# wenxiaoshuai/Points-Matching

Measured on AMD Instinct MI355X. Metric: descriptor-pair distances/s (BF-L2 2-NN + ratio stage); RANSAC hypotheses/s in `ransac`, higher is better.
Workload: dtype f32

## Files before the change

### points_matching_amd/csrc/ransac_a_fused.hip

```cpp
#include "affine_core.hpp"
#include "ransac_fused_kernels.hpp"

namespace pm_ransac {
namespace {

using namespace pm_affine;

constexpr int RA_SYNC_WORD = 12;

template <int MODEL>
struct AModel {
    static constexpr int MIN_PTS = Traits<MODEL>::MIN_PTS;
    static constexpr bool SHARD_OUT = false;
    static constexpr int OUT_WORDS = 6;
    static constexpr bool CANDIDATES = false;

    template <typename DIAG>
    static __device__ __forceinline__ bool solve(const pm_points_view& v, const int* __restrict__ offs, int n, uint64_t seed,
                                                 uint64_t h, double (&A)[9])
    {
        int idx[MIN_PTS];
        sample<MODEL>(seed, h, n, idx);
        double x1[MIN_PTS], y1[MIN_PTS], x2[MIN_PTS], y2[MIN_PTS];
#pragma unroll
        for (int i = 0; i < MIN_PTS; ++i) {
            float2 a, b;
            view_point(v, offs, idx[i], a, b);
            x1[i] = static_cast<double>(a.x); y1[i] = static_cast<double>(a.y);
            x2[i] = static_cast<double>(b.x); y2[i] = static_cast<double>(b.y);
        }
        if constexpr (MODEL == FULL) return solve3(x1, y1, x2, y2, A);
        else return solve2(x1, y1, x2, y2, A);
    }

    static __device__ __forceinline__ void inlier_pk(const ModelS& m, f32x2 x, f32x2 y, f32x2 xp, f32x2 yp, float thr2, bool& ia,
                                                     bool& ib)
    {
        const f32x2 u = sfma_out<0>(m.q03, x, sfma_in<0, 1>(m.q12, y));
        const f32x2 v = sfma_out<1>(m.q03, x, sfma_in<0, 1>(m.q45, y));
        const f32x2 du = u - xp, dv = v - yp;
        const f32x2 lhs = __builtin_elementwise_fma(du, du, dv * dv);
// ... 24 lines not shown
```

### points_matching_amd/csrc/ransac_core.hpp

```cpp
#pragma once
#include "pm_common.hpp"

namespace pm_ransac {

struct NoDiag {
    static constexpr bool scalar_fma = false;
    static __device__ __forceinline__ void phase(int) {}
    static __device__ __forceinline__ void solve(int) {}
};

constexpr int MODEL_STRIDE = 12;

__device__ __forceinline__ uint64_t mix64(uint64_t z)
{
    z = (z ^ (z >> 30)) * 0xBF58476D1CE4E5B9ULL;
    z = (z ^ (z >> 27)) * 0x94D049BB133111EBULL;
    return z ^ (z >> 31);
}

__device__ __forceinline__ void sample8(uint64_t seed, uint64_t h, int n, int (&idx)[8])
{
    const uint64_t stream = mix64(seed ^ 0x9E3779B97F4A7C15ULL) ^ mix64(h + 0xD1B54A32D192ED03ULL);
    int cand[8];
#pragma unroll
    for (int d = 0; d < 8; ++d) {
        const uint64_t r = mix64(stream + static_cast<uint64_t>(d + 1) * 0x9E3779B97F4A7C15ULL);
        cand[d] = static_cast<int>(((r >> 32) * static_cast<uint64_t>(static_cast<uint32_t>(n))) >> 32);
    }
    unsigned dup = 0u;
#pragma unroll
    for (int d = 1; d < 8; ++d)
#pragma unroll
        for (int e = 0; e < d; ++e) dup |= (cand[e] == cand[d] ? 1u : 0u) << d;
#pragma unroll
    for (int s = 0; s < 8; ++s) idx[s] = cand[s];
    if (dup == 0u) return;
#pragma unroll
    for (int s = 0; s < 8; ++s) idx[s] = -1;
    int cnt = 0;
#pragma unroll
    for (int d = 0; d < 8; ++d) {
// ... 315 lines not shown
```

### points_matching_amd/csrc/ransac_e_fused.hip

```cpp
#include "ransac_fused_kernels.hpp"

namespace pm_ransac {
namespace {

constexpr int RE_SYNC_WORD = 16;

struct EModel {
    static constexpr int MIN_PTS = 5;
    static constexpr bool SHARD_OUT = false;
    static constexpr int OUT_WORDS = 9;
    static constexpr bool CANDIDATES = true;

    static __device__ __forceinline__ bool load(const double* __restrict__ cand, int k, double (&E)[9])
    {
        const double* c = cand + 10 * static_cast<size_t>(k);
#pragma unroll
        for (int i = 0; i < 9; ++i) E[i] = c[i];
        return c[9] != 0.0;
    }
    static __device__ __forceinline__ void inlier_pk(const ModelS& m, f32x2 x, f32x2 y, f32x2 xp, f32x2 yp, float thr2, bool& ia,
                                                     bool& ib)
    {
        FModel<PM_ERR_SAMPSON>::inlier_pk(m, x, y, xp, yp, thr2, ia, ib);
    }
    static __device__ __forceinline__ void inlier_x2(const float (&f)[9], f32x2 x, f32x2 y, f32x2 xp, f32x2 yp, float thr2,
                                                     bool& ia, bool& ib)
    {
        FModel<PM_ERR_SAMPSON>::inlier_x2(f, x, y, xp, yp, thr2, ia, ib);
    }
};

}

int ransac_e_enqueue(pm_ctx* ctx, const pm_points_view& vn, const pm_ransac_params* q, const double* d_cand,
                     unsigned long long* d_key, double* d_E, uint8_t* d_mask, int mask_len, int* d_ninl)
{
    return fused_lds_enqueue<EModel>(ctx, vn, q, RE_SYNC_WORD, "ransac_e_fused", d_key, d_E, d_mask, mask_len, d_ninl, d_cand);
}
// ... 3 lines not shown
```

### points_matching_amd/csrc/ransac_fused_kernels.hpp

```cpp
#pragma once
#include <type_traits>

#include "ransac_core.hpp"
#include "ransac_internal.hpp"

namespace pm_ransac {
namespace {

constexpr int RF_THREADS = 256;
constexpr int RF_TEAMS = 2;
constexpr int RF_WG = RF_THREADS * RF_TEAMS;
constexpr int RF_PTS_PER_SLOT = 2 * RF_THREADS;
constexpr int RF_PPT2 = 5;
constexpr int RF_PPT2_BIG = 10;
static_assert(RF_PPT2_BIG <= 10, "score_tile is instantiated for 1..10 slots");

struct RfSlot {
    unsigned long long key;
    double F[9];
    unsigned long long pad[6];
};
static_assert(sizeof(RfSlot) == 128, "slot stride");

struct RfOut {
    int shard;
    unsigned long long* key;
    double* F;
    uint8_t* mask;
    int mask_len;
    int* n_inliers;
    FinalOut* fo;
    union {
        pm_ransac_record* rec;
        const double* cand;
    };
};

// ... 165 lines not shown
            bool ia, ib;
            if constexpr (DIAG::scalar_fma) {
                ia = inlier32<KIND>(fs, X[k][0], Y[k][0], XP[k][0], YP[k][0], thr2);
                ib = inlier32<KIND>(fs, X[k][1], Y[k][1], XP[k][1], YP[k][1], thr2);
            } else {
                inlier_pk_model<KIND>(ms, X[k], Y[k], XP[k], YP[k], thr2, ia, ib);
            }
            va[k] = __ballot(ia);
            vb[k] = __ballot(ib);
        }
        int c = 0;
#pragma unroll
        for (int k = 0; k < KM; ++k) c += __popcll(va[k]) + __popcll(vb[k]);
        if (lane == 0) {
            if (first) cnt[wave][s] = c;
            else __hip_atomic_fetch_add(&cnt[wave][s], c, __ATOMIC_RELAXED, __HIP_MEMORY_SCOPE_WORKGROUP);
        }
    }
}

template <int NWAVES>
__device__ __forceinline__ unsigned long long wg_max_u64(unsigned long long key, unsigned long long* __restrict__ wk, int tid)
{
    key = pm::wave_max_u64(key);
    __syncthreads();
    if ((tid & 63) == 0) wk[tid >> 6] = key;
    __syncthreads();
    unsigned long long k = wk[0];
#pragma unroll
    for (int w = 1; w < NWAVES; ++w) k = wk[w] > k ? wk[w] : k;
    return k;
}

template <int KIND, int PPT2, typename DIAG>
__global__ __launch_bounds__(RF_WG) void ransac_fused(pm_points_view v, uint64_t seed, int64_t hyp_begin, int nh, int hb,
                                                           float thr2, RfSlot* __restrict__ slots, int* __restrict__ ticket,
                                                           RfOut out)
{
    __shared__ __attribute__((aligned(16))) float s_mdl[RF_HB_MAX][12];
    __shared__ double s_m64[RF_HB_MAX][9];
    __shared__ int s_cnt[RF_THREADS / 64][RF_HB_MAX];
    __shared__ int s_offs[PM_MAX_PARTS + 1];
    __shared__ unsigned long long s_wk[RF_WG / 64];
    __shared__ double s_F64[9];
    __shared__ int s_role;
    __shared__ int s_wc[RF_THREADS / 64];

    const int tid = threadIdx.x, lane = tid & 63, wave = tid >> 6;
    const int team = tid / RF_THREADS, ttid = tid % RF_THREADS, twave = wave % (RF_THREADS / 64);
    DIAG::phase(0);
    int n;
    if (v.parts == 1) {
        n = view_count1(v);
    } else {
        view_offsets(v, s_offs, tid);
        __syncthreads();
        n = s_offs[v.parts];
    }
    DIAG::phase(1);

    constexpr int RF_TILE = RF_PTS_PER_SLOT * PPT2;
    const int ntiles = n > RF_TILE ? (n + RF_TILE - 1) / RF_TILE : 1;
    f32x2 X[PPT2], Y[PPT2], XP[PPT2], YP[PPT2];
    const float nanv = __builtin_nanf("");
    auto load_tile = [&](int t) -> int {
        const int base = t * RF_TILE;
        int kmax = (n - base + RF_PTS_PER_SLOT - 1) / RF_PTS_PER_SLOT;
        kmax = kmax < 0 ? 0 : (kmax > PPT2 ? PPT2 : kmax);
#pragma unroll
// ... 24 lines not shown

    const int h0 = static_cast<int>(blockIdx.x) * hb;
    const int hcount = nh - h0 < hb ? nh - h0 : hb;
    if (tid < hcount) {
        double F[9];
        bool ok = false;
#pragma unroll
        for (int i = 0; i < 9; ++i) F[i] = 0.0;
        if (n >= 8) ok = hyp_model_view<DIAG>(v, s_offs, n, seed, static_cast<uint64_t>(hyp_begin + h0 + tid), F);
#pragma unroll
        for (int i = 0; i < 9; ++i) { s_mdl[tid][i] = static_cast<float>(F[i]); s_m64[tid][i] = F[i]; }
        s_mdl[tid][9] = ok ? 1.f : 0.f;
        s_mdl[tid][10] = 0.f; s_mdl[tid][11] = 0.f;
    }
    DIAG::phase(3);
    int kmax = load_tile(0);
    __syncthreads();
    DIAG::phase(4);

    for (int t = 0; t < ntiles; ++t) {
        if (t > 0) kmax = load_tile(t);
        switch (kmax) {
#define PM_CASE(KM_) case KM_: score_tile<KIND, PPT2, (KM_ <= PPT2 ? KM_ : PPT2), DIAG>(s_mdl, s_cnt, hcount, X, Y, XP, YP, thr2, t == 0, lane, twave, team); break;
            PM_CASE(1) PM_CASE(2) PM_CASE(3) PM_CASE(4) PM_CASE(5) PM_CASE(6) PM_CASE(7) PM_CASE(8) PM_CASE(9) PM_CASE(10)
#undef PM_CASE
            default:
                if (team == 0) for (int s = lane; s < hcount; s += 64) s_cnt[twave][s] = t == 0 ? 0 : s_cnt[twave][s];
                break;
        }
    }
    DIAG::phase(5);
    __syncthreads();

    unsigned long long key = 0ull;
    if (tid < hcount && s_mdl[tid][9] != 0.f) {
        int c = 0;
#pragma unroll
        for (int w = 0; w < RF_THREADS / 64; ++w) c += s_cnt[w][tid];
        key = (static_cast<unsigned long long>(static_cast<uint32_t>(c)) << 32) |
              static_cast<unsigned long long>(0xFFFFFFFFu - static_cast<uint32_t>(hyp_begin + h0 + tid));
    }
    const unsigned long long kbest = wg_max_u64<RF_WG / 64>(key, s_wk, tid);
    if (wave == 0) {
        const int sb = kbest ? static_cast<int>(static_cast<int64_t>(0xFFFFFFFFu - static_cast<uint32_t>(kbest)) - hyp_begin) - h0 : 0;
        RfSlot* sl = slots + blockIdx.x;
        if (lane < 9) __hip_atomic_store(&sl->F[lane], kbest ? s_m64[sb][lane] : 0.0, __ATOMIC_RELAXED, __HIP_MEMORY_SCOPE_AGENT);
        if (lane == 9) __hip_atomic_store(&sl->key, kbest, __ATOMIC_RELAXED, __HIP_MEMORY_SCOPE_AGENT);
        asm volatile("s_waitcnt vmcnt(0)" ::: "memory");
        if (lane == 0) {
            const int tk = __hip_atomic_fetch_add(ticket, 1, __ATOMIC_RELAXED, __HIP_MEMORY_SCOPE_AGENT);
            s_role = tk == static_cast<int>(gridDim.x) - 1 ? 1 : 0;
        }
    }
    __syncthreads();
    DIAG::phase(6);
    if (s_role == 0) { DIAG::phase(9); return; }

    if (tid == 0) __hip_atomic_store(ticket, 0, __ATOMIC_RELAXED, __HIP_MEMORY_SCOPE_AGENT);
    unsigned long long kb = 0ull;
    double fb[9];
#pragma unroll
    for (int i = 0; i < 9; ++i) fb[i] = 0.0;
    for (int j = tid; j < static_cast<int>(gridDim.x); j += RF_WG) {
        const unsigned long long kj = __hip_atomic_load(&slots[j].key, __ATOMIC_RELAXED, __HIP_MEMORY_SCOPE_AGENT);
        double fj[9];
#pragma unroll
        for (int i = 0; i < 9; ++i) fj[i] = __hip_atomic_load(&slots[j].F[i], __ATOMIC_RELAXED, __HIP_MEMORY_SCOPE_AGENT);
        if (kj > kb) {
            kb = kj;
#pragma unroll
            for (int i = 0; i < 9; ++i) fb[i] = fj[i];
        }
    }
    const unsigned long long kwin = wg_max_u64<RF_WG / 64>(kb, s_wk, tid);
    const bool ok = kwin != 0ull && n >= 8;
    if (tid < 9) s_F64[tid] = 0.0;
    __syncthreads();
    if (ok && kb == kwin) {
#pragma unroll
        for (int i = 0; i < 9; ++i) s_F64[i] = fb[i];
    }
    __syncthreads();
    DIAG::phase(7);
    if (out.shard) {
        if (tid < 9) out.rec->F[tid] = s_F64[tid];
        if (tid == 9) out.rec->key = ok ? kwin : 0ull;
        return;
    }
    if (tid < 9) {
        if (out.F) out.F[tid] = s_F64[tid];
        if (out.fo) { out.fo->F[tid] = s_F64[tid]; out.fo->F32[tid] = static_cast<float>(s_F64[tid]); }
    }
    if (tid == 9) {
        *out.key = ok ? kwin : 0ull;
        if (out.fo) out.fo->valid = ok ? 1 : 0;
    }
    float fw[9];
#pragma unroll
    for (int i = 0; i < 9; ++i) fw[i] = static_cast<float>(s_F64[i]);
    int mine = 0;
    if (team == 0) {
        for (int t = 0; t < ntiles; ++t) {
            if (ntiles > 1) kmax = load_tile(t);
#pragma unroll
            for (int k = 0; k < PPT2; ++k) {
                if (k < kmax) {
// ... 97 lines not shown
#pragma unroll
            for (int h = 0; h < NH; ++h) s_cnt[ss[h]] += c[h];
        }
    } else {
        ModelS ms[NH];
        int c[NH];
#pragma unroll
        for (int h = 0; h < NH; ++h) {
            const float* m = s_mdl[ss[h]];
            ms[h] = model_to_sgprs(*reinterpret_cast<const f32x4v*>(m), *reinterpret_cast<const f32x4v*>(m + 4),
                                   *reinterpret_cast<const f32x2*>(m + 8));
            c[h] = 0;
        }
        for (int slot = 0; slot < kslots; ++slot) {
            const f32x2 x = pp[0], y = pp[64], xp = pp[128], yp = pp[192];
            pp += 256;
#pragma unroll
            for (int h = 0; h < NH; ++h) {
                bool ia, ib;
                MODEL::inlier_pk(ms[h], x, y, xp, yp, thr2, ia, ib);
                c[h] += __popcll(__ballot(ia)) + __popcll(__ballot(ib));
            }
        }
        if (lane == 0) {
#pragma unroll
            for (int h = 0; h < NH; ++h) s_cnt[ss[h]] += c[h];
        }
    }
}

template <typename MODEL, typename DIAG>
__global__ __launch_bounds__(RL_THREADS) void ransac_fused_lds(pm_points_view v, uint64_t seed, int64_t hyp_begin, int nh, int hb,
                                                               float thr2, int tile_slots, RfSlot* __restrict__ slots,
                                                               int* __restrict__ ticket, RfOut out)
{
    using G = typename GeomOf<MODEL>::type;
    extern __shared__ __attribute__((aligned(16))) f32x2 s_pts[];
    __shared__ __attribute__((aligned(16))) float s_mdl[RF_HB_MAX][G::MW];
    __shared__ double s_m64[RF_HB_MAX][G::WORDS];
    __shared__ int s_cnt[RF_HB_MAX];
    __shared__ int s_offs[PM_MAX_PARTS + 1];
    __shared__ unsigned long long s_wk[RL_WAVES];
    __shared__ double s_F64[G::WORDS];
    __shared__ int s_role;
    __shared__ int s_wc[RL_WAVES];

    const int tid = threadIdx.x, lane = tid & 63, wave = tid >> 6;
    DIAG::phase(0);
    int n;
    if (v.parts == 1) {
        n = view_count1(v);
    } else {
        view_offsets(v, s_offs, tid);
        __syncthreads();
        n = s_offs[v.parts];
    }
    DIAG::phase(1);
    const int tile_pts = tile_slots * RL_SLOT_PTS;
    const int ntiles = n > tile_pts ? (n + tile_pts - 1) / tile_pts : 1;
    const float nanv = __builtin_nanf("");
    auto load_pair = [&](int base, int slot, int l) {
        const int i0 = base + 2 * (64 * slot + l);
        if constexpr (G::OWN) {
            MODEL::load_pair(v, n, i0, s_pts + static_cast<size_t>(slot) * G::PLANES * 64 + l);
        } else {
            float2 a0 = {nanv, nanv}, b0 = a0, a1 = a0, b1 = a0;
            if (v.parts == 1) {
// ... 71 lines not shown
        if constexpr (MODEL::CANDIDATES) {
            const int sk = wave + RL_WAVES * lane;
            unsigned long long live = __ballot(sk < hcount && s_mdl[sk < hcount ? sk : 0][G::FLAG] != 0.f);
            while (live) {
                int ss[4];
                int k = 0;
#pragma unroll
                for (int h = 0; h < 4; ++h) {
                    ss[h] = wave;
                    if (live) {
                        ss[h] = wave + RL_WAVES * static_cast<int>(__builtin_ctzll(live));
                        live &= live - 1;
                        k = h + 1;
                    }
                }
                if (k == 4) score_lds_ids<MODEL, 4, G>(s_mdl, s_cnt, s_pts + lane, kslots, ss, thr2, lane);
                else if (k == 3) score_lds_ids<MODEL, 3, G>(s_mdl, s_cnt, s_pts + lane, kslots, ss, thr2, lane);
                else if (k == 2) score_lds_ids<MODEL, 2, G>(s_mdl, s_cnt, s_pts + lane, kslots, ss, thr2, lane);
                else score_lds_ids<MODEL, 1, G>(s_mdl, s_cnt, s_pts + lane, kslots, ss, thr2, lane);
            }
        } else {
            for (int s = wave; s < hcount; s += 4 * RL_WAVES) {
                const int left = (hcount - s + RL_WAVES - 1) / RL_WAVES;
                if (left >= 4) score_lds<MODEL, 4>(s_mdl, s_cnt, s_pts + lane, kslots, s, thr2, lane);
                else if (left == 3) score_lds<MODEL, 3>(s_mdl, s_cnt, s_pts + lane, kslots, s, thr2, lane);
                else if (left == 2) score_lds<MODEL, 2>(s_mdl, s_cnt, s_pts + lane, kslots, s, thr2, lane);
                else score_lds<MODEL, 1>(s_mdl, s_cnt, s_pts + lane, kslots, s, thr2, lane);
            }
        }
    }
    DIAG::phase(5);
    __syncthreads();

    unsigned long long key = 0ull;
    if (tid < hcount && s_mdl[tid][G::FLAG] != 0.f)
        key = (static_cast<unsigned long long>(static_cast<uint32_t>(s_cnt[tid])) << 32) |
              static_cast<unsigned long long>(0xFFFFFFFFu - static_cast<uint32_t>(hyp_begin + h0 + tid));
    const unsigned long long kbest = wg_max_u64<RL_WAVES>(key, s_wk, tid);
    if (wave == 0) {
        const int sb = kbest ? static_cast<int>(static_cast<int64_t>(0xFFFFFFFFu - static_cast<uint32_t>(kbest)) - hyp_begin) - h0 : 0;
        double* sf = reinterpret_cast<double*>(slots) + static_cast<size_t>(lane) * gridDim.x + blockIdx.x;
        if (lane < G::WORDS) __hip_atomic_store(sf, kbest ? s_m64[sb][lane] : 0.0, __ATOMIC_RELAXED, __HIP_MEMORY_SCOPE_AGENT);
        if (lane == G::WORDS) __hip_atomic_store(reinterpret_cast<unsigned long long*>(sf), kbest, __ATOMIC_RELAXED, __HIP_MEMORY_SCOPE_AGENT);
        asm volatile("s_waitcnt vmcnt(0)" ::: "memory");
        if (lane == 0) {
            const int tk = __hip_atomic_fetch_add(ticket, 1, __ATOMIC_RELAXED, __HIP_MEMORY_SCOPE_AGENT);
            s_role = tk == static_cast<int>(gridDim.x) - 1 ? 1 : 0;
        }
    }
    __syncthreads();
    DIAG::phase(6);
    if (s_role == 0) { DIAG::phase(9); return; }

    if (tid == 0) __hip_atomic_store(ticket, 0, __ATOMIC_RELAXED, __HIP_MEMORY_SCOPE_AGENT);
    unsigned long long kb = 0ull;
    double fb[G::WORDS];
#pragma unroll
    for (int i = 0; i < G::WORDS; ++i) fb[i] = 0.0;
    for (int j = tid; j < static_cast<int>(gridDim.x); j += RL_THREADS) {
        const double* sf = reinterpret_cast<const double*>(slots) + j;
        const unsigned long long kj = __hip_atomic_load(reinterpret_cast<const unsigned long long*>(sf + G::WORDS * static_cast<size_t>(gridDim.x)),
                                                        __ATOMIC_RELAXED, __HIP_MEMORY_SCOPE_AGENT);
        double fj[G::WORDS];
#pragma unroll
        for (int i = 0; i < G::WORDS; ++i) fj[i] = __hip_atomic_load(sf + i * static_cast<size_t>(gridDim.x), __ATOMIC_RELAXED, __HIP_MEMORY_SCOPE_AGENT);
        if (kj > kb) {
            kb = kj;
#pragma unroll
            for (int i = 0; i < G::WORDS; ++i) fb[i] = fj[i];
        }
    }
    const unsigned long long kwin = wg_max_u64<RL_WAVES>(kb, s_wk, tid);
    const bool ok = kwin != 0ull && n >= MODEL::MIN_PTS;
    if (tid < G::WORDS) s_F64[tid] = 0.0;
    __syncthreads();
    if (ok && kb == kwin) {
#pragma unroll
        for (int i = 0; i < G::WORDS; ++i) s_F64[i] = fb[i];
    }
    __syncthreads();
    DIAG::phase(7);
    if (MODEL::SHARD_OUT && out.shard) {
        if (tid < 9) out.rec->F[tid] = s_F64[tid];
        if (tid == 9) out.rec->key = ok ? kwin : 0ull;
        return;
    }
    if (tid < G::WORDS) {
        if (out.F && (MODEL::OUT_WORDS == G::WORDS || tid < MODEL::OUT_WORDS)) out.F[tid] = s_F64[tid];
        if (MODEL::SHARD_OUT && out.fo) { out.fo->F[tid] = s_F64[tid]; out.fo->F32[tid] = static_cast<float>(s_F64[tid]); }
    }
    if (tid == G::WORDS) {
        *out.key = ok ? kwin : 0ull;
        if (MODEL::SHARD_OUT && out.fo) out.fo->valid = ok ? 1 : 0;
    }
    float fw[G::OWN ? G::MW : 9];
    if constexpr (G::OWN) {
        MODEL::mask_model(out.cand, ok, kwin, hyp_begin, fw);
    } else {
#pragma unroll
        for (int i = 0; i < 9; ++i) fw[i] = static_cast<float>(s_F64[i]);
    }
    int mine = 0;
    for (int t = 0; t < ntiles; ++t) {
        const int kslots = tile_kslots(t);
        if (ntiles > 1) {
            __syncthreads();
            for (int slot = wave; slot < kslots; slot += RL_WAVES) load_pair(t * tile_pts, slot, lane);
            __syncthreads();
        }
        for (int slot = wave; slot < kslots; slot += RL_WAVES) {
            const f32x2* pp = s_pts + static_cast<size_t>(slot) * (64 * G::PLANES) + lane;
            bool ia, ib;
            if constexpr (G::OWN) {
                f32x2 op[G::PLANES];
#pragma unroll
                for (int q = 0; q < G::PLANES; ++q) op[q] = pp[64 * q];
                MODEL::inlier_x2(fw, op, thr2, ia, ib);
            } else {
                MODEL::inlier_x2(fw, pp[0], pp[64], pp[128], pp[192], thr2, ia, ib);
            }
            ia = ia && ok; ib = ib && ok;
            const int i0 = t * tile_pts + 2 * (64 * slot + lane);
            if (i0 < out.mask_len) out.mask[i0] = ia ? 1 : 0;
            if (i0 + 1 < out.mask_len) out.mask[i0 + 1] = ib ? 1 : 0;
            mine += __popcll(__ballot(ia)) + __popcll(__ballot(ib));
        }
    }
    if (lane == 0) s_wc[wave] = mine;
    const int covered = n > 0 ? (n + RL_SLOT_PTS - 1) / RL_SLOT_PTS * RL_SLOT_PTS : 0;
    for (int i = covered + tid; i < out.mask_len; i += RL_THREADS) out.mask[i] = 0;
    __syncthreads();
    if (tid == 0) {
        int tot = 0;
#pragma unroll
        for (int w = 0; w < RL_WAVES; ++w) tot += s_wc[w];
        if (out.n_inliers) *out.n_inliers = tot;
        if (MODEL::SHARD_OUT && out.fo) out.fo->n_inliers = tot;
    }
    DIAG::phase(8);
    DIAG::phase(9);
}

int sync_words(pm_ctx* ctx, int** out)
{
    if (!ctx->sync_words) {
        PM_HIP_CHECK(hipMalloc(reinterpret_cast<void**>(&ctx->sync_words), 256));
        PM_HIP_CHECK(hipMemsetAsync(ctx->sync_words, 0, 256, ctx->stream));
    }
    *out = ctx->sync_words;
    return PM_OK;
}

template <typename MODEL, typename DIAG>
int fused_lds_launch(pm_ctx* ctx, const pm_points_view& v, const pm_ransac_params* p, int nwg, int hb, RfSlot* slots,
                     int* ticket, const RfOut& out)
{
    using G = typename GeomOf<MODEL>::type;
    const long long cap_total = static_cast<long long>(v.parts) * v.cap;
    const long long need = (cap_total + RL_SLOT_PTS - 1) / RL_SLOT_PTS;
    const int tile_slots = static_cast<int>(need < 1 ? 1 : (need > G::MAX_SLOTS ? G::MAX_SLOTS : need));
    const size_t lds = static_cast<size_t>(tile_slots) * G::PLANES * 64 * sizeof(f32x2);
    static bool attr_done_dev[PM_MAX_DEVICES] = {};
    if (!attr_done_dev[ctx->device]) {
        PM_HIP_CHECK(hipFuncSetAttribute(reinterpret_cast<const void*>(&ransac_fused_lds<MODEL, DIAG>),
                                         hipFuncAttributeMaxDynamicSharedMemorySize,
                                         G::MAX_SLOTS * G::PLANES * 64 * static_cast<int>(sizeof(f32x2))));
        attr_done_dev[ctx->device] = true;
    }
    const float thr2 = p->thresh_px * p->thresh_px;
    hipLaunchKernelGGL((ransac_fused_lds<MODEL, DIAG>), dim3(nwg), dim3(RL_THREADS), lds, ctx->stream, v, p->seed, p->hyp_begin,
                       static_cast<int>(p->hyp_end - p->hyp_begin), hb, thr2, tile_slots, slots, ticket, out);
    PM_HIP_CHECK(hipGetLastError());
    return PM_OK;
}

template <typename MODEL>
int fused_lds_enqueue(pm_ctx* ctx, const pm_points_view& v, const pm_ransac_params* p, int sync_word, const char* timer,
                      unsigned long long* d_key, double* d_model, uint8_t* d_mask, int mask_len, int* d_ninl,
                      const double* d_cand = nullptr)
{
    const long long nh = p->hyp_end - p->hyp_begin;
    const int hb = fused_hb(ctx, nh);
    const int nwg = static_cast<int>((nh + hb - 1) / hb);
    RfSlot* slots = static_cast<RfSlot*>(pm::arena_take(ctx, sizeof(RfSlot) * static_cast<size_t>(nwg)));
    PM_REQUIRE(slots, PM_E_NOMEM, "scratch arena too small");
    int* sync = nullptr;
    int rc = sync_words(ctx, &sync);
    if (rc != PM_OK) return rc;
    RfOut out{};
    out.key = d_key; out.F = d_model; out.mask = d_mask; out.mask_len = mask_len; out.n_inliers = d_ninl;
    out.cand = d_cand;
    pm::ScopedKernelTime t(ctx, timer);
    return fused_lds_launch<MODEL, NoDiag>(ctx, v, p, nwg, hb, slots, sync + sync_word, out);
}

template <typename DIAG>
int fused_launch_t(pm_ctx* ctx, const pm_points_view& v, const pm_ransac_params* p, int shard, pm_ransac_record* d_rec,
                 unsigned long long* d_key, double* d_F, uint8_t* d_mask, int mask_len, int* d_ninl, FinalOut** fo_out)
{
    const long long nh = p->hyp_end - p->hyp_begin;
    const long long cap_total = static_cast<long long>(v.parts) * v.cap;
    PM_REQUIRE(nh >= 1, PM_E_INVALID, "fused_launch: empty hypothesis range");
    PM_REQUIRE(nh <= 0x7FFFFFFFLL, PM_E_INVALID, "a single launch takes at most 2^31 - 1 hypothesis ids: split the range");
    const int hb = fused_hb(ctx, nh);
    const int nwg = static_cast<int>((nh + hb - 1) / hb);
    RfSlot* slots = static_cast<RfSlot*>(pm::arena_take(ctx, sizeof(RfSlot) * static_cast<size_t>(nwg)));
    FinalOut* fo = static_cast<FinalOut*>(pm::arena_take(ctx, sizeof(FinalOut)));
    PM_REQUIRE(slots && fo, PM_E_NOMEM, "scratch arena too small");
    int* sync = nullptr;
    int rc = sync_words(ctx, &sync);
    if (rc != PM_OK) return rc;
    RfOut out{};
    out.shard = shard;
    out.key = d_key; out.F = d_F; out.mask = d_mask; out.mask_len = mask_len; out.n_inliers = d_ninl;
    out.fo = fo_out ? fo : nullptr;
    out.rec = d_rec;
    if (fo_out) *fo_out = fo;
    const float thr2 = p->thresh_px * p->thresh_px;
    pm::ScopedKernelTime t(ctx, "ransac_fused");
    if (ctx->opts[PM_OPT_RANSAC_FORM] != 1) {
        if (p->error_kind == PM_ERR_SAMPSON) return fused_lds_launch<FModel<PM_ERR_SAMPSON>, DIAG>(ctx, v, p, nwg, hb, slots, sync, out);
        return fused_lds_launch<FModel<PM_ERR_SYM_EPIPOLAR>, DIAG>(ctx, v, p, nwg, hb, slots, sync, out);
    }
#define PM_RF(KIND_, PPT2_)                                                                                              \
    hipLaunchKernelGGL((ransac_fused<KIND_, PPT2_, DIAG>), dim3(nwg), dim3(RF_WG), 0, ctx->stream, v, p->seed, p->hyp_begin, \
                       static_cast<int>(nh), hb, thr2, slots, sync, out)
    const int depth = cap_total <= 2 * RF_PTS_PER_SLOT ? 2 : (cap_total <= RF_PPT2 * RF_PTS_PER_SLOT ? RF_PPT2 : RF_PPT2_BIG);
#define PM_RF_K(KIND_)                                                                   \
    do {                                                                                 \
        if (depth == 2) PM_RF(KIND_, 2);                                                 \
        else if (depth == RF_PPT2) PM_RF(KIND_, RF_PPT2);                                \
        else PM_RF(KIND_, RF_PPT2_BIG);                                                  \
    } while (0)
    if (p->error_kind == PM_ERR_SAMPSON) PM_RF_K(PM_ERR_SAMPSON);
    else PM_RF_K(PM_ERR_SYM_EPIPOLAR);
#undef PM_RF_K
#undef PM_RF
    PM_HIP_CHECK(hipGetLastError());
    return PM_OK;
}

}
}
```

### points_matching_amd/csrc/ransac_h_fused.hip

```cpp
#include "homography_core.hpp"
#include "ransac_fused_kernels.hpp"

namespace pm_ransac {
namespace {

using namespace pm_homog;

constexpr int RH_SYNC_WORD = 8;

struct HModel {
    static constexpr int MIN_PTS = 4;
    static constexpr bool SHARD_OUT = false;
    static constexpr int OUT_WORDS = 9;
    static constexpr bool CANDIDATES = false;

    template <typename DIAG>
    static __device__ __forceinline__ bool solve(const pm_points_view& v, const int* __restrict__ offs, int n, uint64_t seed,
                                                 uint64_t h, double (&H)[9])
    {
        int idx[4];
        sample4(seed, h, n, idx);
        double x1[4], y1[4], x2[4], y2[4];
#pragma unroll
        for (int i = 0; i < 4; ++i) {
            float2 a, b;
            view_point(v, offs, idx[i], a, b);
            x1[i] = static_cast<double>(a.x); y1[i] = static_cast<double>(a.y);
            x2[i] = static_cast<double>(b.x); y2[i] = static_cast<double>(b.y);
        }
        return solve4(x1, y1, x2, y2, H);
    }

    static __device__ __forceinline__ void inlier_pk(const ModelS& m, f32x2 x, f32x2 y, f32x2 xp, f32x2 yp, float thr2, bool& ia,
                                                     bool& ib)
    {
        const f32x2 u = sfma_out<0>(m.q03, x, sfma_in<0, 1>(m.q12, y));
        const f32x2 v = sfma_out<1>(m.q03, x, sfma_in<0, 1>(m.q45, y));
        const f32x2 w = sfma_out<1>(m.q36, x, sfma_in<0, 1>(m.q78, y));
        const f32x2 du = __builtin_elementwise_fma(-xp, w, u);
        const f32x2 dv = __builtin_elementwise_fma(-yp, w, v);
        const f32x2 lhs = __builtin_elementwise_fma(du, du, dv * dv);
// ... 22 lines not shown
```

### points_matching_amd/csrc/ransac_p_fused.hip

```cpp
#include "pnp_core.hpp"
#include "ransac_fused_kernels.hpp"

namespace pm_ransac {
namespace {

using pm_pnp::SLOT_DOUBLES;

constexpr int RP_SYNC_WORD = 20;

struct PnpGeom {
    static constexpr bool OWN = true;
    static constexpr int PLANES = 5, MW = 16, FLAG = 12, WORDS = 12, MAX_SLOTS = 48;
};

__device__ __forceinline__ bool inlier1(const float (&P)[16], float x, float y, float z, float u, float v, float thr2)
{
    const float a = fmaf(P[0], x, fmaf(P[1], y, fmaf(P[2], z, P[3])));
    const float b = fmaf(P[4], x, fmaf(P[5], y, fmaf(P[6], z, P[7])));
    const float w = fmaf(P[8], x, fmaf(P[9], y, fmaf(P[10], z, P[11])));
    const float du = fmaf(-u, w, a), dv = fmaf(-v, w, b);
    const float lhs = fmaf(du, du, dv * dv), rhs = thr2 * (w * w);
    return lhs <= rhs && w > 0.0f && rhs > 0.0f && rhs < __builtin_inff();
}

struct PModel {
    using Geom = PnpGeom;
    static constexpr int MIN_PTS = 4;
    static constexpr bool SHARD_OUT = false;
    static constexpr int OUT_WORDS = 12;
    static constexpr bool CANDIDATES = true;

    struct Regs {
        unsigned long long q01, q23, q45, q67, q89, qab;
    };
    static __device__ __forceinline__ Regs regs(const float* m)
    {
        return Regs{spair(m[0], m[1]), spair(m[2], m[3]), spair(m[4], m[5]), spair(m[6], m[7]), spair(m[8], m[9]),
                    spair(m[10], m[11])};
    }

    static __device__ __forceinline__ bool load(const double* __restrict__ cand, int k, double (&F)[12], float* mdl)
// ... 70 lines not shown
```

### points_matching_amd/csrc/ransac_shard.hip

```cpp
#include "ransac_fused_kernels.hpp"

namespace pm_ransac {
namespace {

template <int KIND>
__global__ __launch_bounds__(RF_THREADS) void ransac_finish(pm_points_view v, const pm_ransac_record* __restrict__ recs, int nrec,
                                                            float thr2, unsigned long long* __restrict__ key_out,
                                                            double* __restrict__ F_out, uint8_t* __restrict__ mask, int mask_len,
                                                            int* __restrict__ n_inl_out, int* __restrict__ n_total_out,
                                                            int* __restrict__ sync)
{
    __shared__ int s_offs[PM_MAX_PARTS + 1];
    __shared__ unsigned long long s_wk[RF_THREADS / 64];
    __shared__ int s_wc[RF_THREADS / 64];
    __shared__ int s_last;
    const int tid = threadIdx.x, lane = tid & 63, wave = tid >> 6;
    if (v.parts > 1) view_offsets(v, s_offs, tid);
    unsigned long long kb = 0ull;
    for (int j = tid; j < nrec; j += RF_THREADS) { const unsigned long long kj = recs[j].key; kb = kj > kb ? kj : kb; }
    const unsigned long long kwin = wg_max_u64<RF_THREADS / 64>(kb, s_wk, tid);
    const int n = v.parts > 1 ? s_offs[v.parts] : view_count1(v);
    const bool ok = kwin != 0ull && n >= 8;
    int owner = 0;
    for (int j = 0; j < nrec; ++j) owner = recs[j].key == kwin ? j : owner;
// ... 71 lines not shown
    PM_REQUIRE(ctx != nullptr && d_record != nullptr && p != nullptr, PM_E_INVALID, "null argument");
    int rc = check_view(view);
    if (rc != PM_OK) return rc;
    PM_REQUIRE(p->hyp_begin >= 0 && p->hyp_end > p->hyp_begin && p->hyp_end <= 0x100000000LL, PM_E_INVALID,
               "hypothesis ids must satisfy 0 <= begin < end <= 2^32");
    PM_REQUIRE(p->error_kind == PM_ERR_SAMPSON || p->error_kind == PM_ERR_SYM_EPIPOLAR, PM_E_INVALID, "unknown error_kind");
    PM_HIP_CHECK(hipSetDevice(ctx->device));
    rc = pm::arena_reserve(ctx, fused_scratch_bytes(ctx, p) + 1024);
    if (rc != PM_OK) return rc;
    pm::arena_reset(ctx);
    return fused_launch(ctx, *view, p, 1, d_record, nullptr, nullptr, nullptr, 0, nullptr, nullptr);
}

extern "C" int pm_ransac_finish_parts_dev(pm_ctx* ctx, const pm_points_view* view, const pm_ransac_params* p,
                                          const pm_ransac_record* d_records, int n_records, uint64_t* d_key, double* d_F,
                                          uint8_t* d_mask, int mask_len, int32_t* d_n_inliers, int32_t* d_n_total)
{
    PM_REQUIRE(ctx != nullptr && p != nullptr && d_records != nullptr && d_mask != nullptr, PM_E_INVALID, "null argument");
    PM_REQUIRE(n_records >= 1 && mask_len >= 0, PM_E_INVALID, "need n_records >= 1, mask_len >= 0");
    int rc = check_view(view);
    if (rc != PM_OK) return rc;
    PM_REQUIRE(p->error_kind == PM_ERR_SAMPSON || p->error_kind == PM_ERR_SYM_EPIPOLAR, PM_E_INVALID, "unknown error_kind");
    PM_HIP_CHECK(hipSetDevice(ctx->device));
    int* sync = nullptr;
    rc = sync_words(ctx, &sync);
    if (rc != PM_OK) return rc;
    const float thr2 = p->thresh_px * p->thresh_px;
    int blocks = (mask_len + 8 * RF_THREADS - 1) / (8 * RF_THREADS);
    blocks = blocks < 1 ? 1 : (blocks > 64 ? 64 : blocks);
    pm::ScopedKernelTime t(ctx, "ransac_finish");
    unsigned long long* key = reinterpret_cast<unsigned long long*>(d_key);
    if (p->error_kind == PM_ERR_SAMPSON)
        hipLaunchKernelGGL(ransac_finish<PM_ERR_SAMPSON>, dim3(blocks), dim3(RF_THREADS), 0, ctx->stream, *view, d_records,
                           n_records, thr2, key, d_F, d_mask, mask_len, d_n_inliers, d_n_total, sync + 2);
    else
        hipLaunchKernelGGL(ransac_finish<PM_ERR_SYM_EPIPOLAR>, dim3(blocks), dim3(RF_THREADS), 0, ctx->stream, *view, d_records,
                           n_records, thr2, key, d_F, d_mask, mask_len, d_n_inliers, d_n_total, sync + 2);
    PM_HIP_CHECK(hipGetLastError());
    return PM_OK;
}
```

Baseline: 2268 billion.

## Use two-level cache-line-padded completion tickets and trim RANSAC fused-kernel tail

Replaces the single global atomic ticket with a two-level ticket scheme: workgroups first arrive on one of eight per-group counters, each on its own cache line, and only group finishers touch the root counter. The goal is less atomic contention on one word when many workgroups finish. Each model family's sync words are also padded apart, so different families no longer share cache lines. The per-workgroup best-key reduction now runs in wave 0 only, dropping a workgroup-wide reduction and its barriers. The final mask writes use paired 16-bit stores and vectorised zero fill. In exchange there are more sync bytes, extra atomics for the last arriver, and reset logic spread over multiple words.

```diff
diff --git a/points_matching_amd/csrc/ransac_a_fused.hip b/points_matching_amd/csrc/ransac_a_fused.hip
--- a/points_matching_amd/csrc/ransac_a_fused.hip
+++ b/points_matching_amd/csrc/ransac_a_fused.hip
@@ -6,7 +6,6 @@
 
 using namespace pm_affine;
 
-constexpr int RA_SYNC_WORD = 12;
 
 template <int MODEL>
 struct AModel {
diff --git a/points_matching_amd/csrc/ransac_core.hpp b/points_matching_amd/csrc/ransac_core.hpp
--- a/points_matching_amd/csrc/ransac_core.hpp
+++ b/points_matching_amd/csrc/ransac_core.hpp
@@ -7,6 +7,7 @@
     static constexpr bool scalar_fma = false;
     static __device__ __forceinline__ void phase(int) {}
     static __device__ __forceinline__ void solve(int) {}
+    static __device__ __forceinline__ void tail(int) {}
 };
 
 constexpr int MODEL_STRIDE = 12;
diff --git a/points_matching_amd/csrc/ransac_e_fused.hip b/points_matching_amd/csrc/ransac_e_fused.hip
--- a/points_matching_amd/csrc/ransac_e_fused.hip
+++ b/points_matching_amd/csrc/ransac_e_fused.hip
@@ -3,7 +3,6 @@
 namespace pm_ransac {
 namespace {
 
-constexpr int RE_SYNC_WORD = 16;
 
 struct EModel {
     static constexpr int MIN_PTS = 5;
diff --git a/points_matching_amd/csrc/ransac_fused_kernels.hpp b/points_matching_amd/csrc/ransac_fused_kernels.hpp
--- a/points_matching_amd/csrc/ransac_fused_kernels.hpp
+++ b/points_matching_amd/csrc/ransac_fused_kernels.hpp
@@ -3,6 +3,7 @@
 
 #include "ransac_core.hpp"
 #include "ransac_internal.hpp"
+#include "ransac_ticket.hpp"
 
 namespace pm_ransac {
 namespace {
@@ -234,9 +235,43 @@
     return k;
 }
 
+template <typename KEYOF>
+__device__ __forceinline__ unsigned long long wave0_max_key(int hcount, int lane, KEYOF key_of)
+{
+    static_assert(RF_HB_MAX <= 128, "two ids per lane");
+    unsigned long long k = 0ull;
+    if (lane < hcount) k = key_of(lane);
+    if (lane + 64 < hcount) { const unsigned long long k1 = key_of(lane + 64); k = k1 > k ? k1 : k; }
+    return pm::wave_max_u64(k);
+}
+
+__device__ __forceinline__ int* ticket_word(int* sync, int i) { return sync + i * RT_LINE_WORDS; }
+template <typename DIAG>
+__device__ __forceinline__ bool arrive_is_last(int* __restrict__ sync)
+{
+    const int nwg = static_cast<int>(gridDim.x), ng = ticket_groups(nwg);
+    bool last;
+    if (ng == 1) {
+        last = __hip_atomic_fetch_add(ticket_word(sync, 0), 1, __ATOMIC_RELAXED, __HIP_MEMORY_SCOPE_AGENT) == nwg - 1;
+        DIAG::tail(2);
+    } else {
+        const int g = static_cast<int>(blockIdx.x) % ng;
+        last = __hip_atomic_fetch_add(ticket_word(sync, 1 + g), 1, __ATOMIC_RELAXED, __HIP_MEMORY_SCOPE_AGENT) ==
+               ticket_group_size(nwg, ng, g) - 1;
+        DIAG::tail(2);
+        if (last) last = __hip_atomic_fetch_add(ticket_word(sync, 0), 1, __ATOMIC_RELAXED, __HIP_MEMORY_SCOPE_AGENT) == ng - 1;
+    }
+    DIAG::tail(3);
+    return last;
+}
+__device__ __forceinline__ void ticket_reset(int* __restrict__ sync, int tid)
+{
+    if (tid <= RT_GROUPS) __hip_atomic_store(ticket_word(sync, tid), 0, __ATOMIC_RELAXED, __HIP_MEMORY_SCOPE_AGENT);
+}
+
 template <int KIND, int PPT2, typename DIAG>
 __global__ __launch_bounds__(RF_WG) void ransac_fused(pm_points_view v, uint64_t seed, int64_t hyp_begin, int nh, int hb,
-                                                           float thr2, RfSlot* __restrict__ slots, int* __restrict__ ticket,
+                                                           float thr2, RfSlot* __restrict__ slots, int* __restrict__ sync,
                                                            RfOut out)
 {
     __shared__ __attribute__((aligned(16))) float s_mdl[RF_HB_MAX][12];
@@ -327,31 +362,28 @@
     DIAG::phase(5);
     __syncthreads();
 
-    unsigned long long key = 0ull;
-    if (tid < hcount && s_mdl[tid][9] != 0.f) {
-        int c = 0;
-#pragma unroll
-        for (int w = 0; w < RF_THREADS / 64; ++w) c += s_cnt[w][tid];
-        key = (static_cast<unsigned long long>(static_cast<uint32_t>(c)) << 32) |
-              static_cast<unsigned long long>(0xFFFFFFFFu - static_cast<uint32_t>(hyp_begin + h0 + tid));
-    }
-    const unsigned long long kbest = wg_max_u64<RF_WG / 64>(key, s_wk, tid);
     if (wave == 0) {
+        const unsigned long long kbest = wave0_max_key(hcount, lane, [&](int s) {
+            if (s_mdl[s][9] == 0.f) return 0ull;
+            int c = 0;
+#pragma unroll
+            for (int w = 0; w < RF_THREADS / 64; ++w) c += s_cnt[w][s];
+            return (static_cast<unsigned long long>(static_cast<uint32_t>(c)) << 32) |
+                   static_cast<unsigned long long>(0xFFFFFFFFu - static_cast<uint32_t>(hyp_begin + h0 + s));
+        });
+        DIAG::tail(0);
         const int sb = kbest ? static_cast<int>(static_cast<int64_t>(0xFFFFFFFFu - static_cast<uint32_t>(kbest)) - hyp_begin) - h0 : 0;
         RfSlot* sl = slots + blockIdx.x;
         if (lane < 9) __hip_atomic_store(&sl->F[lane], kbest ? s_m64[sb][lane] : 0.0, __ATOMIC_RELAXED, __HIP_MEMORY_SCOPE_AGENT);
         if (lane == 9) __hip_atomic_store(&sl->key, kbest, __ATOMIC_RELAXED, __HIP_MEMORY_SCOPE_AGENT);
         asm volatile("s_waitcnt vmcnt(0)" ::: "memory");
-        if (lane == 0) {
-            const int tk = __hip_atomic_fetch_add(ticket, 1, __ATOMIC_RELAXED, __HIP_MEMORY_SCOPE_AGENT);
-            s_role = tk == static_cast<int>(gridDim.x) - 1 ? 1 : 0;
-        }
+        DIAG::tail(1);
+        if (lane == 0) s_role = arrive_is_last<DIAG>(sync) ? 1 : 0;
     }
     __syncthreads();
     DIAG::phase(6);
     if (s_role == 0) { DIAG::phase(9); return; }
 
-    if (tid == 0) __hip_atomic_store(ticket, 0, __ATOMIC_RELAXED, __HIP_MEMORY_SCOPE_AGENT);
     unsigned long long kb = 0ull;
     double fb[9];
 #pragma unroll
@@ -367,6 +399,7 @@
             for (int i = 0; i < 9; ++i) fb[i] = fj[i];
         }
     }
+    ticket_reset(sync, tid);
     const unsigned long long kwin = wg_max_u64<RF_WG / 64>(kb, s_wk, tid);
     const bool ok = kwin != 0ull && n >= 8;
     if (tid < 9) s_F64[tid] = 0.0;
@@ -530,7 +563,7 @@
 template <typename MODEL, typename DIAG>
 __global__ __launch_bounds__(RL_THREADS) void ransac_fused_lds(pm_points_view v, uint64_t seed, int64_t hyp_begin, int nh, int hb,
                                                                float thr2, int tile_slots, RfSlot* __restrict__ slots,
-                                                               int* __restrict__ ticket, RfOut out)
+                                                               int* __restrict__ sync, RfOut out)
 {
     using G = typename GeomOf<MODEL>::type;
     extern __shared__ __attribute__((aligned(16))) f32x2 s_pts[];
@@ -668,27 +701,25 @@
     DIAG::phase(5);
     __syncthreads();
 
-    unsigned long long key = 0ull;
-    if (tid < hcount && s_mdl[tid][G::FLAG] != 0.f)
-        key = (static_cast<unsigned long long>(static_cast<uint32_t>(s_cnt[tid])) << 32) |
-              static_cast<unsigned long long>(0xFFFFFFFFu - static_cast<uint32_t>(hyp_begin + h0 + tid));
-    const unsigned long long kbest = wg_max_u64<RL_WAVES>(key, s_wk, tid);
     if (wave == 0) {
+        const unsigned long long kbest = wave0_max_key(hcount, lane, [&](int s) {
+            return s_mdl[s][G::FLAG] == 0.f ? 0ull
+                                            : (static_cast<unsigned long long>(static_cast<uint32_t>(s_cnt[s])) << 32) |
+                                                  static_cast<unsigned long long>(0xFFFFFFFFu - static_cast<uint32_t>(hyp_begin + h0 + s));
+        });
+        DIAG::tail(0);
         const int sb = kbest ? static_cast<int>(static_cast<int64_t>(0xFFFFFFFFu - static_cast<uint32_t>(kbest)) - hyp_begin) - h0 : 0;
         double* sf = reinterpret_cast<double*>(slots) + static_cast<size_t>(lane) * gridDim.x + blockIdx.x;
         if (lane < G::WORDS) __hip_atomic_store(sf, kbest ? s_m64[sb][lane] : 0.0, __ATOMIC_RELAXED, __HIP_MEMORY_SCOPE_AGENT);
         if (lane == G::WORDS) __hip_atomic_store(reinterpret_cast<unsigned long long*>(sf), kbest, __ATOMIC_RELAXED, __HIP_MEMORY_SCOPE_AGENT);
         asm volatile("s_waitcnt vmcnt(0)" ::: "memory");
-        if (lane == 0) {
-            const int tk = __hip_atomic_fetch_add(ticket, 1, __ATOMIC_RELAXED, __HIP_MEMORY_SCOPE_AGENT);
-            s_role = tk == static_cast<int>(gridDim.x) - 1 ? 1 : 0;
-        }
+        DIAG::tail(1);
+        if (lane == 0) s_role = arrive_is_last<DIAG>(sync) ? 1 : 0;
     }
     __syncthreads();
     DIAG::phase(6);
     if (s_role == 0) { DIAG::phase(9); return; }
 
-    if (tid == 0) __hip_atomic_store(ticket, 0, __ATOMIC_RELAXED, __HIP_MEMORY_SCOPE_AGENT);
     unsigned long long kb = 0ull;
     double fb[G::WORDS];
 #pragma unroll
@@ -706,11 +737,19 @@
             for (int i = 0; i < G::WORDS; ++i) fb[i] = fj[i];
         }
     }
-    const unsigned long long kwin = wg_max_u64<RL_WAVES>(kb, s_wk, tid);
+    DIAG::tail(4);
+    ticket_reset(sync, tid);
+    const unsigned long long kwave = pm::wave_max_u64(kb);
+    if (lane == 0) s_wk[wave] = kwave;
+    __syncthreads();
+    unsigned long long kwin = s_wk[0];
+#pragma unroll
+    for (int w = 1; w < RL_WAVES; ++w) kwin = s_wk[w] > kwin ? s_wk[w] : kwin;
+    DIAG::tail(5);
     const bool ok = kwin != 0ull && n >= MODEL::MIN_PTS;
-    if (tid < G::WORDS) s_F64[tid] = 0.0;
-    __syncthreads();
-    if (ok && kb == kwin) {
+    if (!ok) {
+        if (tid < G::WORDS) s_F64[tid] = 0.0;
+    } else if (kb == kwin) {
 #pragma unroll
         for (int i = 0; i < G::WORDS; ++i) s_F64[i] = fb[i];
     }
@@ -736,6 +775,7 @@
 #pragma unroll
         for (int i = 0; i < 9; ++i) fw[i] = static_cast<float>(s_F64[i]);
     }
+    const bool mask_pairs = (reinterpret_cast<uintptr_t>(out.mask) & 1) == 0;
     int mine = 0;
     for (int t = 0; t < ntiles; ++t) {
         const int kslots = tile_kslots(t);
@@ -757,14 +797,29 @@
             }
             ia = ia && ok; ib = ib && ok;
             const int i0 = t * tile_pts + 2 * (64 * slot + lane);
-            if (i0 < out.mask_len) out.mask[i0] = ia ? 1 : 0;
-            if (i0 + 1 < out.mask_len) out.mask[i0 + 1] = ib ? 1 : 0;
+            if (i0 + 1 < out.mask_len && mask_pairs) {
+                *reinterpret_cast<uint16_t*>(out.mask + i0) = static_cast<uint16_t>((ia ? 1 : 0) | (ib ? 0x100 : 0));
+            } else {
+                if (i0 < out.mask_len) out.mask[i0] = ia ? 1 : 0;
+                if (i0 + 1 < out.mask_len) out.mask[i0 + 1] = ib ? 1 : 0;
+            }
             mine += __popcll(__ballot(ia)) + __popcll(__ballot(ib));
         }
     }
     if (lane == 0) s_wc[wave] = mine;
     const int covered = n > 0 ? (n + RL_SLOT_PTS - 1) / RL_SLOT_PTS * RL_SLOT_PTS : 0;
-    for (int i = covered + tid; i < out.mask_len; i += RL_THREADS) out.mask[i] = 0;
+    if (covered < out.mask_len) {
+        uint8_t* zb = out.mask + covered;
+        const int zlen = out.mask_len - covered;
+        int head = static_cast<int>((16 - (reinterpret_cast<uintptr_t>(zb) & 15)) & 15);
+        head = head < zlen ? head : zlen;
+        const int nvec = (zlen - head) / 16;
+        uint4* zv = reinterpret_cast<uint4*>(zb + head);
+        if (tid < head) zb[tid] = 0;
+        for (int i = tid; i < nvec; i += RL_THREADS) zv[i] = uint4{0u, 0u, 0u, 0u};
+        const int tail0 = head + 16 * nvec;
+        if (tail0 + tid < zlen) zb[tail0 + tid] = 0;
+    }
     __syncthreads();
     if (tid == 0) {
         int tot = 0;
@@ -780,8 +835,8 @@
 int sync_words(pm_ctx* ctx, int** out)
 {
     if (!ctx->sync_words) {
-        PM_HIP_CHECK(hipMalloc(reinterpret_cast<void**>(&ctx->sync_words), 256));
-        PM_HIP_CHECK(hipMemsetAsync(ctx->sync_words, 0, 256, ctx->stream));
+        PM_HIP_CHECK(hipMalloc(reinterpret_cast<void**>(&ctx->sync_words), RT_SYNC_BYTES));
+        PM_HIP_CHECK(hipMemsetAsync(ctx->sync_words, 0, RT_SYNC_BYTES, ctx->stream));
     }
     *out = ctx->sync_words;
     return PM_OK;
@@ -789,7 +844,7 @@
 
 template <typename MODEL, typename DIAG>
 int fused_lds_launch(pm_ctx* ctx, const pm_points_view& v, const pm_ransac_params* p, int nwg, int hb, RfSlot* slots,
-                     int* ticket, const RfOut& out)
+                     int* sync, const RfOut& out)
 {
     using G = typename GeomOf<MODEL>::type;
     const long long cap_total = static_cast<long long>(v.parts) * v.cap;
@@ -805,7 +860,7 @@
     }
     const float thr2 = p->thresh_px * p->thresh_px;
     hipLaunchKernelGGL((ransac_fused_lds<MODEL, DIAG>), dim3(nwg), dim3(RL_THREADS), lds, ctx->stream, v, p->seed, p->hyp_begin,
-                       static_cast<int>(p->hyp_end - p->hyp_begin), hb, thr2, tile_slots, slots, ticket, out);
+                       static_cast<int>(p->hyp_end - p->hyp_begin), hb, thr2, tile_slots, slots, sync, out);
     PM_HIP_CHECK(hipGetLastError());
     return PM_OK;
 }
@@ -855,12 +910,12 @@
     const float thr2 = p->thresh_px * p->thresh_px;
     pm::ScopedKernelTime t(ctx, "ransac_fused");
     if (ctx->opts[PM_OPT_RANSAC_FORM] != 1) {
-        if (p->error_kind == PM_ERR_SAMPSON) return fused_lds_launch<FModel<PM_ERR_SAMPSON>, DIAG>(ctx, v, p, nwg, hb, slots, sync, out);
-        return fused_lds_launch<FModel<PM_ERR_SYM_EPIPOLAR>, DIAG>(ctx, v, p, nwg, hb, slots, sync, out);
+        if (p->error_kind == PM_ERR_SAMPSON) return fused_lds_launch<FModel<PM_ERR_SAMPSON>, DIAG>(ctx, v, p, nwg, hb, slots, sync + RF_SYNC_WORD, out);
+        return fused_lds_launch<FModel<PM_ERR_SYM_EPIPOLAR>, DIAG>(ctx, v, p, nwg, hb, slots, sync + RF_SYNC_WORD, out);
     }
 #define PM_RF(KIND_, PPT2_)                                                                                              \
     hipLaunchKernelGGL((ransac_fused<KIND_, PPT2_, DIAG>), dim3(nwg), dim3(RF_WG), 0, ctx->stream, v, p->seed, p->hyp_begin, \
-                       static_cast<int>(nh), hb, thr2, slots, sync, out)
+                       static_cast<int>(nh), hb, thr2, slots, sync + RF_SYNC_WORD, out)
     const int depth = cap_total <= 2 * RF_PTS_PER_SLOT ? 2 : (cap_total <= RF_PPT2 * RF_PTS_PER_SLOT ? RF_PPT2 : RF_PPT2_BIG);
 #define PM_RF_K(KIND_)                                                                   \
     do {                                                                                 \
diff --git a/points_matching_amd/csrc/ransac_h_fused.hip b/points_matching_amd/csrc/ransac_h_fused.hip
--- a/points_matching_amd/csrc/ransac_h_fused.hip
+++ b/points_matching_amd/csrc/ransac_h_fused.hip
@@ -6,7 +6,6 @@
 
 using namespace pm_homog;
 
-constexpr int RH_SYNC_WORD = 8;
 
 struct HModel {
     static constexpr int MIN_PTS = 4;
diff --git a/points_matching_amd/csrc/ransac_p_fused.hip b/points_matching_amd/csrc/ransac_p_fused.hip
--- a/points_matching_amd/csrc/ransac_p_fused.hip
+++ b/points_matching_amd/csrc/ransac_p_fused.hip
@@ -6,7 +6,6 @@
 
 using pm_pnp::SLOT_DOUBLES;
 
-constexpr int RP_SYNC_WORD = 20;
 
 struct PnpGeom {
     static constexpr bool OWN = true;
diff --git a/points_matching_amd/csrc/ransac_shard.hip b/points_matching_amd/csrc/ransac_shard.hip
--- a/points_matching_amd/csrc/ransac_shard.hip
+++ b/points_matching_amd/csrc/ransac_shard.hip
@@ -127,10 +127,10 @@
     unsigned long long* key = reinterpret_cast<unsigned long long*>(d_key);
     if (p->error_kind == PM_ERR_SAMPSON)
         hipLaunchKernelGGL(ransac_finish<PM_ERR_SAMPSON>, dim3(blocks), dim3(RF_THREADS), 0, ctx->stream, *view, d_records,
-                           n_records, thr2, key, d_F, d_mask, mask_len, d_n_inliers, d_n_total, sync + 2);
+                           n_records, thr2, key, d_F, d_mask, mask_len, d_n_inliers, d_n_total, sync + RFIN_SYNC_WORD);
     else
         hipLaunchKernelGGL(ransac_finish<PM_ERR_SYM_EPIPOLAR>, dim3(blocks), dim3(RF_THREADS), 0, ctx->stream, *view, d_records,
-                           n_records, thr2, key, d_F, d_mask, mask_len, d_n_inliers, d_n_total, sync + 2);
+                           n_records, thr2, key, d_F, d_mask, mask_len, d_n_inliers, d_n_total, sync + RFIN_SYNC_WORD);
     PM_HIP_CHECK(hipGetLastError());
     return PM_OK;
 }
diff --git a/points_matching_amd/csrc/ransac_ticket.hpp b/points_matching_amd/csrc/ransac_ticket.hpp
--- /dev/null
+++ b/points_matching_amd/csrc/ransac_ticket.hpp
@@ -0,0 +1,27 @@
+#pragma once
+
+#if defined(__HIPCC__)
+#define PM_TICKET_HD __host__ __device__
+#else
+#define PM_TICKET_HD
+#endif
+
+namespace pm_ransac {
+
+constexpr int RT_GROUPS = 8;
+constexpr int RT_TWO_LEVEL_MIN = 64;
+constexpr int RT_LINE_WORDS = 32;
+constexpr int RT_FAMILY_WORDS = (1 + RT_GROUPS) * RT_LINE_WORDS;
+
+constexpr int RF_SYNC_WORD = 0 * RT_FAMILY_WORDS;
+constexpr int RH_SYNC_WORD = 1 * RT_FAMILY_WORDS;
+constexpr int RA_SYNC_WORD = 2 * RT_FAMILY_WORDS;
+constexpr int RE_SYNC_WORD = 3 * RT_FAMILY_WORDS;
+constexpr int RP_SYNC_WORD = 4 * RT_FAMILY_WORDS;
+constexpr int RFIN_SYNC_WORD = 5 * RT_FAMILY_WORDS;
+constexpr int RT_SYNC_BYTES = (RFIN_SYNC_WORD + RT_LINE_WORDS) * static_cast<int>(sizeof(int));
+
+PM_TICKET_HD inline int ticket_groups(int nwg) { return nwg < RT_TWO_LEVEL_MIN ? 1 : RT_GROUPS; }
+PM_TICKET_HD inline int ticket_group_size(int nwg, int ng, int g) { return (nwg - g + ng - 1) / ng; }
+
+}
```

After: 2280 billion, median of 3. No clear change (+0.5%).
